# DeepMETv2/DeepMETv2

Measured on AMD Instinct MI355X. Metric: events/sec (4.5k PF cands, k=16), higher is better.
Workload: dtype f32

## Files before the change

deepmetv2_amd/_lib.py:

```python
from __future__ import annotations

import ctypes as C
import os
import threading

_PKG_DIR = os.path.dirname(os.path.abspath(__file__))
LIB_PATH = os.environ.get("DMET_HIP_LIB") or os.path.join(_PKG_DIR, "libdmet_hip.so")

_lock = threading.Lock()
_lib = None

_vp, _i, _i64, _sz, _f, _d = C.c_void_p, C.c_int, C.c_int64, C.c_size_t, C.c_float, C.c_double

SIGNATURES = {
    "dmet_version": (_i, []),
    "dmet_last_error": (C.c_char_p, []),
    "dmet_device_available": (_i, []),
    "dmet_knn_workspace_bytes": (_sz, [_i64, _i, _i, _i]),
    "dmet_knn_f32": (_i, [_vp, _vp, _i, _i64, _i, _i, _vp, _vp, _vp, _sz, _vp]),
    "dmet_knn_local_f32": (_i, [_vp, _vp, _i, _i64, _i, _i, _vp, _vp, _vp, _vp, _sz, _vp]),
    "dmet_knn_periodic_f32": (_i, [_vp, _vp, _i, _i64, _i, _i, _vp, _vp, _vp, _vp, _vp, _sz, _vp]),
    "dmet_knn_xy_workspace_bytes": (_sz, [_i64, _i64, _i, _i, _i]),
    "dmet_knn_xy_f32": (_i, [_vp, _vp, _i64, _vp, _vp, _i64, _i, _i, _i, _vp, _vp, _vp, _vp, _sz, _vp]),
    "dmet_radius_xy_f32": (_i, [_vp, _vp, _i64, _vp, _vp, _i64, _i, _i, _f, _i, _vp, _i, _vp, _vp, _vp]),
    "dmet_edge_features_xy_f32": (_i, [_vp, _vp, _vp, _vp, _i64, _i, _vp, _vp]),
    "dmet_edge_features_xy_bwd_f32": (_i, [_vp, _vp, _vp, _vp, _i64, _i64, _i, _vp, _vp, _vp]),
    "dmet_adamw_f32": (_i, [_vp, _vp, _vp, _vp, _vp, _vp, _i64, _d, _d, _d, _d, _d, _vp]),
    "dmet_adamw_lr_f32": (_i, [_vp, _vp, _vp, _vp, _vp, _vp, _i64, _vp, _d, _d, _d, _d, _vp]),
    "dmet_bn_knn_local_dense_f32": (_i, [_vp, _vp, _vp, _vp, _vp, _vp, _vp, _vp, _i, _i64, _i, _i, _vp, _vp, _vp, _vp, _vp, _i,
                                         _vp, _vp, _vp, _vp, _vp, _sz, _vp]),
    "dmet_knn_local_dense_f32": (_i, [_vp, _vp, _i, _i64, _i, _i, _vp, _vp, _vp, _vp, _vp, _i, _vp, _vp, _vp, _vp, _sz, _vp]),
    "dmet_knn_fallback_stats": (_i, [_vp, _i64, _i, _i, _i, _vp, _vp]),
    "dmet_knn_size_hint": (_i, [_i, _i]),
    "dmet_finalize_defer_begin": (_i, []),
    "dmet_finalize_pending": (_i, []),
    "dmet_finalize_flush": (_i, [_vp]),
    "dmet_radius_f32": (_i, [_vp, _vp, _i, _i64, _i, _f, _i, _i, _vp, _vp, _vp]),
    "dmet_radius_counted_f32": (_i, [_vp, _vp, _i, _i64, _i, _f, _i, _i, _vp, _vp, _vp]),
    "dmet_radius_workspace_bytes": (_sz, [_i64]),
    "dmet_radius_windowed_f32": (_i, [_vp, _vp, _i, _i64, _i, _f, _i, _i, _i, _vp, _vp, _vp, _sz, _vp]),
    "dmet_radius_windowed_local_f32": (_i, [_vp, _vp, _i, _i64, _i, _f, _i, _i, _i, _vp, _vp, _vp, _i, _vp, _sz, _vp]),
    "dmet_radius_periodic_f32": (_i, [_vp, _vp, _i, _i64, _i, _f, _i, _i, _i, _vp, _vp, _vp, _vp]),
    "dmet_radius_windowed_periodic_f32": (_i, [_vp, _vp, _i, _i64, _i, _f, _i, _i, _i, _vp, _vp, _vp, _vp, _i, _vp, _sz,
                                               _vp]),
    "dmet_edgeconv_linear_workspace_bytes": (_sz, [_i64, _i]),
    "dmet_edgeconv_linear_max_fwd_f32": (_i, [_vp, _vp, _vp, _i, _i64, _i, _i, _i, _vp, _vp, _vp, _vp, _vp, _sz, _vp]),
    "dmet_edgeconv_fused_lds_f32": (_i, [_vp, _vp, _vp, _i, _i64, _i, _i, _i, _vp, _vp, _vp, _vp, _vp]),
    "dmet_node_linear_split_f32": (_i, [_vp, _i64, _i, _i, _vp, _vp, _vp, _vp, _vp]),
    "dmet_node_linear_split_sliced_f32": (_i, [_vp, _i64, _i, _i, _vp, _vp, _vp, _vp, _vp]),
    "dmet_bn_node_linear_split_f32": (_i, [_vp, _vp, _vp, _vp, _vp, _vp, _vp, _i64, _i, _vp, _vp, _i, _vp, _vp, _vp]),
    "dmet_gather_max_f32": (_i, [_vp, _vp, _vp, _vp, _i, _i64, _i, _i, _vp, _vp, _vp]),
    "dmet_gather_max_counted_f32": (_i, [_vp, _vp, _vp, _vp, _i64, _i, _i, _vp, _vp, _vp]),
    "dmet_gather_max_lds_f32": (_i, [_vp, _vp, _vp, _vp, _i, _i64, _i, _i, _vp, _vp, _vp]),
    "dmet_gather_max_counted_lds_f32": (_i, [_vp, _vp, _vp, _vp, _vp, _i, _i64, _i, _i, _i, _vp, _vp, _vp]),
    "dmet_gather_max_lds_sliced_f32": (_i, [_vp, _vp, _vp, _vp, _vp, _i, _i64, _i, _i, _vp, _vp, _vp]),
    "dmet_gather_max_lds_sliced_cap_f32": (_i, [_vp, _vp, _vp, _vp, _vp, _i, _i64, _i, _i, _vp, _vp, _i64, _vp]),
    "dmet_gather_max_lds16_f32": (_i, [_vp, _vp, _vp, _vp, _vp, _i, _i64, _i, _i, _vp, _vp, _vp]),
    "dmet_edge_mlp2_supported": (_i, [_i, _i, _i, _i]),
    "dmet_edge_mlp2_bf16": (_i, [_vp, _i64, _i, _vp, _i, _vp, _vp, _i, _vp, _vp, _i, _i, _i, _vp, _vp]),
    "dmet_edge_mlp2_bn_workspace_bytes": (_sz, [_i64, _i]),
    "dmet_edge_mlp2_bn_bf16": (_i, [_vp, _i64, _i, _vp, _i, _vp, _vp, _i, _vp, _vp, _i, _i, _i, _vp, _vp, _f, _f, _vp, _vp, _vp,
                                    _i, _vp, _vp, _sz, _vp]),
    "dmet_edge_mlp_f32_supported": (_i, [_i, _i, _i]),
    "dmet_edge_mlp_f32_workspace_bytes": (_sz, [_i64, _i64, _i, _i, _i]),
    "dmet_edge_mlp_fwd_f32": (_i, [_vp, _i64, _i, _vp, _vp, _vp, _i64, _vp, _vp, _i, _vp, _vp, _i, _i, _i, _i, _vp, _vp, _f, _f,
# ... 121 lines not shown
```

deepmetv2_amd/_native.py:

```python
from __future__ import annotations

import contextlib
import ctypes
import inspect
import os
from typing import Optional, Tuple

import torch

from . import _lib


def _require_device(*tensors: torch.Tensor) -> torch.device:
    dev = None
    for t in tensors:
        if t is None:
            continue
        if t.device.type != "cuda":
            raise RuntimeError(
                "deepmetv2_amd: operator called with a non-GPU tensor. The HIP extension is the only "
                "implementation (no CPU fallback); move inputs to a ROCm device.")
        if dev is None:
            dev = t.device
        elif t.device != dev:
# ... 164 lines not shown
        dense = None

    def call(nbr, dist, loc_p, ws):
        if dense is None:
            _lib.check(L.dmet_knn_local_f32(x.data_ptr(), ptr.data_ptr(), B, N, D, k, nbr.data_ptr(), dist.data_ptr(),
                                            loc_p, ws.data_ptr(), ws.numel(), _stream(dev)), "dmet_knn_local_f32")
            return None
        W, b, sliced = dense
        W = _f32c(W.detach(), "W")
        bp = _f32c(b.detach(), "b").data_ptr() if b is not None else None
        if sliced == "bf16":
            Pt = torch.empty((N, 32), dtype=torch.float32, device=dev)
            Qt = torch.empty((N, 32), dtype=torch.bfloat16, device=dev)
            layout = 2
        else:
            PQ = torch.empty((2, 4, N, 8) if sliced else (2, N, 32), dtype=torch.float32, device=dev)
            Pt, Qt = PQ[0], PQ[1]
            layout, sliced = (1 if sliced else 0), bool(sliced)
        done = ctypes.c_int(0)
        _lib.check(L.dmet_knn_local_dense_f32(x.data_ptr(), ptr.data_ptr(), B, N, D, k, nbr.data_ptr(),
                                              dist.data_ptr(), loc_p, W.data_ptr(), bp, layout, Pt.data_ptr(),
                                              Qt.data_ptr(), ctypes.cast(ctypes.pointer(done), ctypes.c_void_p),
                                              ws.data_ptr(), ws.numel(), _stream(dev)), "dmet_knn_local_dense_f32")
        return (Pt, Qt, sliced) if done.value else None

    nbr, dist, loc, ws, pq = _knn_run(dev, N, k, want_local, L.dmet_knn_workspace_bytes(N, B, D, k), call)
    if stats is not None and N > 0 and B > 0:
        with _on(dev):
            out = (ctypes.c_int64 * 2)()
            _lib.check(L.dmet_knn_fallback_stats(ws.data_ptr(), N, B, D, k, ctypes.cast(out, ctypes.c_void_p),
                                                 _stream(dev)), "dmet_knn_fallback_stats")
            stats["flagged_tiles"], stats["flagged_queries"] = int(out[0]), int(out[1])
            stats["tiles"] = (N + 127) // 128
    if asked:
        return nbr, dist, loc, pq
    return nbr, dist, loc


def knn(x: torch.Tensor, ptr: torch.Tensor, k: int, stats: Optional[dict] = None) -> Tuple[torch.Tensor, torch.Tensor]:
    nbr, dist, _ = _knn(x, ptr, k, stats, False)
    return nbr, dist


def knn_local_dense(x: torch.Tensor, ptr: torch.Tensor, k: int, W: torch.Tensor, b: Optional[torch.Tensor],
                    sliced, stats: Optional[dict] = None):
    out = _knn(x, ptr, k, stats, True, dense=(W, b, sliced))
    return out if len(out) == 4 else (*out, None)


def knn_local(x: torch.Tensor, ptr: torch.Tensor, k: int, stats: Optional[dict] = None
              ) -> Tuple[torch.Tensor, torch.Tensor, torch.Tensor]:
    return _knn(x, ptr, k, stats, True)


def _period_array(period, D: int):
    if period is None:
        return None, None
    if len(period) != D:
        raise ValueError(f"period has {len(period)} entries for {D} coordinates")
    per = (ctypes.c_float * D)(*[float(p) for p in period])
    return per, ctypes.cast(per, ctypes.c_void_p)


def knn_periodic(x: torch.Tensor, ptr: torch.Tensor, k: int, period, want_local: bool):
    dev, x, N, D, B = _knn_operands(x, ptr)
    L = _lib.load()
# ... 1569 lines not shown
```

deepmetv2_amd/csrc/knn.hip:

```cpp
#include <stdlib.h>

#include "common.h"
#include "knn_common.h"
#include "nls_body.h"

namespace dmet {
namespace {

constexpr int kTileC = 32;
constexpr int kQMax = 8;
constexpr int kMaxSplit = 8;
constexpr int kWavesPerGroup = 4;

#define DMET_PKSUB_LO " op_sel:[0,0] op_sel_hi:[0,1] neg_lo:[0,1] neg_hi:[0,1]\n\t"
#define DMET_PKSUB_HI " op_sel:[1,0] op_sel_hi:[1,1] neg_lo:[0,1] neg_hi:[0,1]\n\t"
__device__ __forceinline__ void pk_dist_step4(f2 &accA, f2 &accB, f2 vxy, f2 vzw, f2 wxy, f2 wzw, f2 q0, f2 q1, f2 q2,
                                              f2 q3)
{
    f2 t0, t1, t2, t3;
    asm("v_pk_add_f32 %[t0], %[vxy], %[q0]" DMET_PKSUB_LO
        "v_pk_add_f32 %[t1], %[wxy], %[q0]" DMET_PKSUB_LO
        "v_pk_add_f32 %[t2], %[vxy], %[q1]" DMET_PKSUB_HI
        "v_pk_add_f32 %[t3], %[wxy], %[q1]" DMET_PKSUB_HI
        "v_pk_fma_f32 %[a], %[t0], %[t0], %[a]\n\t"
// ... 824 lines not shown
        w.fplan = reinterpret_cast<KnnPlan *>(take(sizeof(KnnPlan)));
        w.forder = reinterpret_cast<int32_t *>(take(sizeof(int32_t) * ((size_t)B + 1)));
        w.fpos_of = reinterpret_cast<int32_t *>(take(sizeof(int32_t) * ((size_t)B + 1)));
        w.ftile_ptr = reinterpret_cast<int32_t *>(take(sizeof(int32_t) * ((size_t)B + 1)));
        w.nrm = reinterpret_cast<float *>(take(sizeof(float) * (size_t)N));
        w.nrec = (N >> 5) + B + 1;
        w.rec = reinterpret_cast<uint8_t *>(take((size_t)w.nrec * kRecBytesMax));
        w.zero_bytes = sizeof(int32_t) * ((size_t)exact_tiles_max(N, B) + 4) + (size_t)N;
        w.flags = reinterpret_cast<int32_t *>(take(w.zero_bytes));
        w.any = w.flags + exact_tiles_max(N, B);
        w.qflag = reinterpret_cast<uint8_t *>(w.any + 4);
        w.qlist = reinterpret_cast<int32_t *>(take(sizeof(int32_t) * (size_t)N));
    }
    w.bytes = (size_t)(p - reinterpret_cast<uintptr_t>(ws));
    return w;
}

inline int filter_mode()
{
    const char *e = getenv("DMET_KNN_PATH");
    if (e && strcmp(e, "exact") == 0) return 0;
#if defined(DMET_KNN_EXPERIMENT) || defined(DMET_FILTER_ABL) || defined(DMET_F2_ABL) || defined(DMET_F2_SAMEREC)
    if (e && strcmp(e, "filter_only") == 0) return 2;
#endif
    return 1;
}

inline int filter_form2()
{
    const char *e = getenv("DMET_KNN_FILTER");
    return (e && strcmp(e, "1") == 0) ? 0 : 1;
}

template <int KF, int NH = 1>
int launch_filter(const KnnFilterArgs &f, const KnnWorkspace &w, int simds, const KnnPlanOut &px, const KnnPlanOut &pf,
                  hipStream_t st, const KnnRider *rider, const KnnAffine *affine)
{
    const int slots = simds * kF2WavesPerSimd;
    if (affine) {
        if constexpr (NH == 1)
            hipLaunchKernelGGL((knn_prep_kernel<1, true>), dim3((unsigned)((w.nrec * kWave + 255) / 256 + 2)), dim3(256), 0, st, f.x,
                               f.ptr, f.B, f.N, w.nrm, w.rec, w.nrec, reinterpret_cast<uint32_t *>(w.flags), w.zero_bytes, px,
                               pf, f.form2, *affine);
    } else {
        hipLaunchKernelGGL((knn_prep_kernel<NH>), dim3((unsigned)((w.nrec * kWave + 255) / 256 + 2)), dim3(256), 0, st, f.x,
                           f.ptr, f.B, f.N, w.nrm, w.rec, w.nrec, reinterpret_cast<uint32_t *>(w.flags), w.zero_bytes, px, pf,
                           f.form2, KnnAffine{});
    }
    DMET_LAUNCH_CHECK("knn_prep_kernel");
    const int64_t ftiles_max = (f.N + kFQ - 1) / kFQ + f.B;
    const int64_t fblocks = (ftiles_max + slots + kWavesPerGroup - 1) / kWavesPerGroup;
    if (f.form2) {
        KnnFilterArgs fr = f;
        int64_t grid = fblocks;
        if (rider) {
            fr.rW = rider->W; fr.rb = rider->b; fr.rP = rider->P; fr.rQ = rider->Q; fr.r_sliced = rider->sliced;
            fr.first_rider = (int)fblocks;
            grid = fblocks + rider_groups();
        }
        hipLaunchKernelGGL((knn_filter12_kernel<KF, NH>), dim3((unsigned)grid), dim3(kWave * kWavesPerGroup), 0, st, fr);
        DMET_LAUNCH_CHECK("knn_filter12_kernel");
    } else {
        if constexpr (NH == 1) hipLaunchKernelGGL((knn_filter_kernel<KF>), dim3((unsigned)fblocks), dim3(kWave * kWavesPerGroup), 0, st, f);
        DMET_LAUNCH_CHECK("knn_filter_kernel");
    }
    constexpr int kRerankQpb = 4 * (kWave / filter_list_len(KF));
// ... 29 lines not shown

template <int DP, int KP>
KnnOutcome launch_knn(const KnnBuild &r, const KnnWorkspace &w)
{
    KnnOutcome done;
    constexpr int TQ = (DP <= 32) ? 2 : 1;
    constexpr int QT = kWave * TQ;
    const KnnQuerySet *qs = r.qs.qx ? &r.qs : nullptr;
    int simds = num_simds();
    if (simds > kMaxSimds) simds = kMaxSimds;
    bool use_filter = false;
    if constexpr ((DP == 32 || DP == 64) && KP <= 32)
        use_filter = !qs && r.D == DP && r.k <= 20 && aligned16(r.x) && filter_mode() != 0 && (DP == 32 || filter_form2());
    constexpr int NH = DP == 64 ? 2 : 1;
    const int slots = simds * kF2WavesPerSimd;
    const KnnPlanOut px{QT, simds, kMaxSplit, w.order, w.pos_of, w.tile_ptr, w.plan};
    const KnnPlanOut pf{kFQ, slots, kFilterMaxSplit, w.forder, w.fpos_of, w.ftile_ptr, w.fplan};
    if (qs) {
        hipLaunchKernelGGL(knn_plan_xy_kernel, dim3(1), dim3(256), 0, r.st, qs->qptr, r.ptr, r.B, px);
        DMET_LAUNCH_CHECK("knn_plan_xy_kernel");
    } else if (!use_filter) {
        hipLaunchKernelGGL(knn_plan_kernel, dim3(1), dim3(256), 0, r.st, r.ptr, r.B, px, pf);
        DMET_LAUNCH_CHECK("knn_plan_kernel");
    }
    KnnArgs a{r.x, r.ptr, r.B, r.N, r.D, r.k, r.nbr, r.dist, r.nbr16, w.wsd, w.wsj, w.plan, w.order, w.tile_ptr, w.psd, w.psj,
              nullptr, 0, nullptr, nullptr, nullptr, 0, QT};
    if (!qs && !use_filter && hipMemsetAsync(w.flags, 0, w.zero_bytes, r.st) != hipSuccess)
        return hip_fail(hipGetLastError(), "hipMemsetAsync");

    if (use_filter) {
        KnnFilterArgs f{r.x, r.ptr, r.B, r.N, r.k, w.nrm, w.rec, w.fplan, w.forder, w.fpos_of, w.ftile_ptr,
                        w.psd, w.psj, r.nbr, r.dist, r.nbr16, w.flags, w.any, w.qflag, w.qlist, w.tile_ptr, QT, filter_form2(),
                        NH == 1 ? 1.0f : 1.5f, nullptr, nullptr, nullptr, nullptr, 0, 0,
                        (aligned16(r.nbr) && aligned16(r.dist) && aligned16(r.nbr16) && !env_is("DMET_KNN_EMIT", "lanes")) ? 1 : 0, 0};
        f.no_rerank = (f.form2 && r.hint.min_nodes >= kF2MinNodes && r.hint.max_nodes >= r.hint.min_nodes &&
                       r.hint.max_nodes <= kF2MaxNodes) ? 1 : 0;
        const KnnAffine *affine = (NH == 1 && r.affine.raw) ? &r.affine : nullptr;
        const KnnRider *rider = (NH == 1 && f.form2 && r.rider.P) ? &r.rider : nullptr;
        int rc = 0;
        if constexpr (DP == 32 || DP == 64) {
            if constexpr (KP == 8) rc = launch_filter<8, NH>(f, w, simds, px, pf, r.st, rider, affine);
            else if constexpr (KP == 16) rc = launch_filter<16, NH>(f, w, simds, px, pf, r.st, rider, affine);
            else if constexpr (KP == 32) rc = launch_filter<20, NH>(f, w, simds, px, pf, r.st, rider, affine);
        }
        if (rc) return rc;
        done.affine_done = affine != nullptr;
        done.rider_done = rider != nullptr;
        if (filter_mode() == 2) return done;
        a.flags = w.flags;
        a.any = w.any;
        if constexpr (NH == 1) {
            a.qlist = w.qlist;
            a.pos_of = w.pos_of;
            a.requery_groups = kRequeryGroups;
            a.flag_min = kRequeryMax + 1;
        } else {
            a.flag_min = 1;
        }
    }

    const int64_t tiles_max = (r.N + QT - 1) / QT + r.B;
    const int64_t blocks = (tiles_max + simds + kWavesPerGroup - 1) / kWavesPerGroup + a.requery_groups;
    unsigned dyn = 0;
#ifdef DMET_KNN_EXPERIMENT
    if (const char *e = getenv("DMET_KNN_EXTRA_LDS")) dyn = (unsigned)atoi(e);
#endif
    const bool exact_d = r.D == DP && aligned16(r.x) && (!qs || aligned16(qs->qx));
// ... 173 lines not shown
    }
    *fused = (o.rc == 0) ? 1 : 0;
    return o.rc;
}

extern "C" int dmet_knn_fallback_stats(const void *ws, int64_t N, int B, int D, int k, int64_t *out, dmet_stream_t stream)
{
    (void)D;
    DMET_REQUIRE(N > 0 && B > 0 && k >= 1 && k <= DMET_MAX_K && ws && out, "dmet_knn_fallback_stats: bad arguments");
    const KnnWorkspace w = carve_workspace(const_cast<void *>(ws), N, B, padded_k(k));
    const int64_t n = exact_tiles_max(N, B);
    int32_t *host = static_cast<int32_t *>(malloc(sizeof(int32_t) * (size_t)n));
    DMET_REQUIRE(host != nullptr, "dmet_knn_fallback_stats: out of host memory");
    hipStream_t st = as_stream(stream);
    hipError_t e = hipMemcpyAsync(host, w.flags, sizeof(int32_t) * (size_t)n, hipMemcpyDeviceToHost, st);
    if (e == hipSuccess) e = hipStreamSynchronize(st);
    if (e != hipSuccess) { free(host); return hip_fail(e, "dmet_knn_fallback_stats"); }
    out[0] = 0; out[1] = 0;
    for (int64_t i = 0; i < n; ++i) { out[0] += host[i] != 0; out[1] += host[i]; }
    free(host);
    if (getenv("DMET_KNN_LIST_FLAGGED") && out[1] > 0) {
        int32_t ids[16];
        const int64_t m = out[1] < 16 ? out[1] : 16;
        if (hipMemcpy(ids, w.qlist, sizeof(int32_t) * (size_t)m, hipMemcpyDeviceToHost) == hipSuccess)
            for (int64_t i = 0; i < m; ++i) {
                uint8_t why = 0;
                (void)hipMemcpy(&why, w.qflag + ids[i], 1, hipMemcpyDeviceToHost);
                fprintf(stderr, "[dmet] flagged query %d (qflag %d)\n", ids[i], (int)why);
            }
    }
    return 0;
}

extern "C" size_t dmet_knn_xy_workspace_bytes(int64_t Nx, int64_t Ny, int B, int D, int k)
{
    (void)Nx; (void)D;
    if (Ny <= 0 || B < 0 || k <= 0 || k > DMET_MAX_K) return 0;
    return carve_workspace(nullptr, Ny, B, padded_k(k), true).bytes + 512;
}

extern "C" int dmet_knn_xy_f32(const float *x, const int64_t *ptr_x, int64_t Nx, const float *y, const int64_t *ptr_y,
                               int64_t Ny, int B, int D, int k, const float *period, int32_t *nbr, float *dist, void *ws,
                               size_t ws_bytes, dmet_stream_t stream)
{
    const int64_t kMaxRows = (int64_t)2147483647 - 4096;
    DMET_REQUIRE(Nx >= 0 && Nx < kMaxRows && Ny >= 0 && Ny < kMaxRows, "dmet_knn_xy_f32: Nx=%lld / Ny=%lld out of range",
                 (long long)Nx, (long long)Ny);
    DMET_REQUIRE(B >= 0, "dmet_knn_xy_f32: B=%d", B);
    DMET_REQUIRE(k >= 1 && k <= DMET_MAX_K, "dmet_knn_xy_f32: k=%d not in [1,%d]", k, DMET_MAX_K);
    DMET_REQUIRE(D >= 1 && D <= DMET_MAX_KNN_DIM, "dmet_knn_xy_f32: D=%d not in [1,%d]", D, DMET_MAX_KNN_DIM);
    RadPeriod per;
    bool any = false;
    if (period) {
        const int rc = radius_periods("dmet_knn_xy_f32", D, period, &per, &any);
        if (rc) return rc;
    }
    if (Ny == 0) return 0;
    DMET_REQUIRE(B >= 1, "dmet_knn_xy_f32: %lld queries but no event", (long long)Ny);
    DMET_REQUIRE((x || Nx == 0) && ptr_x && y && ptr_y && nbr && dist && ws, "dmet_knn_xy_f32: null pointer");
    DMET_REQUIRE(ws_bytes >= dmet_knn_xy_workspace_bytes(Nx, Ny, B, D, k), "dmet_knn_xy_f32: workspace too small");
    return knn_build(KnnBuild{x, ptr_x, Ny, KnnQuerySet{y, ptr_y}, any ? &per : nullptr, B, D, k, nbr, dist, nullptr, ws,
                              ws_bytes, as_stream(stream), KnnRider{}, KnnAffine{}, KnnSizeHint{}}).rc;
}
```

deepmetv2_amd/csrc/knn_filter.h:

```cpp
constexpr int kFQ = 64;

typedef float f32x16 __attribute__((ext_vector_type(16)));
typedef short bf16x8 __attribute__((ext_vector_type(8)));
typedef _Float16 f16x8 __attribute__((ext_vector_type(8)));

struct KnnFilterArgs {
    const float *x;
    const int64_t *ptr;
    int B;
    int64_t N;
    int k;
    float *nrm;
    uint8_t *rec;
    const KnnPlan *plan;
    const int32_t *order;
    const int32_t *pos_of;
    const int32_t *tile_ptr;
    float *psd;
    int32_t *psj;
    int32_t *nbr;
    float *dist;
    uint16_t *nbr16;
    int32_t *flags;
    int32_t *any;
    uint8_t *qflag;
    int32_t *qlist;
    const int32_t *xtile_ptr;
    int xtile_queries;
    int form2;
    float slack_scale;
    const float *rW, *rb;
    float *rP, *rQ;
    int r_sliced;
    int first_rider;
    int emit_coalesced;
    int no_rerank;
};

struct KnnRider {
    const float *W = nullptr, *b = nullptr;
    float *P = nullptr, *Q = nullptr;
    int sliced = 0;
};

struct KnnAffine {
    const float *raw = nullptr, *res = nullptr, *gamma = nullptr, *beta = nullptr, *mean = nullptr, *invstd = nullptr;
    int kernarg_pad = 0;
};
static_assert(sizeof(KnnAffine) == 56, "KnnAffine is the tail of knn_prep_kernel's argument block: keep its size");

inline int rider_groups()
{
    static int cached = 0;
    if (cached == 0) {
        const char *e = getenv("DMET_KNN_RIDER_GROUPS");
        const int v = e ? atoi(e) : 0;
        cached = (v >= 1 && v <= 4096) ? v : 512;
    }
    return cached;
}

__device__ __forceinline__ void flag_query(const KnnFilterArgs &a, int q, int xtile)
{
    a.qflag[q] = 1;
    atomicAdd(a.flags + xtile, 1);
    const int slot = atomicAdd(a.any, 1);
    if (slot < a.N) a.qlist[slot] = q;
}

// ... 682 lines not shown

__device__ __forceinline__ unsigned f2_tau16(float tau, float &rep)
{
    const float x = __builtin_amdgcn_fmed3f(-tau * (1.0f / kF2TauC[0]), -65504.0f, 65504.0f);
    float v = __builtin_amdgcn_fmed3f(__builtin_fmaf(__builtin_fabsf(x), -0x1p-9f, x), -65504.0f, 65504.0f);
    const float y0 = (float)__builtin_amdgcn_cvt_pkrtz(v, v)[0];
    const float w = __builtin_fmaf(-y0, kF2TauC[0] / kF2TauC[1], x * (kF2TauC[0] / kF2TauC[1]));
    v = fminf(__builtin_fmaf(__builtin_fabsf(w), -0x1p-9f, w - 0x1p-24f), 65504.0f);
    const auto y = __builtin_amdgcn_cvt_pkrtz(y0, v);
    rep = -__builtin_fmaf(y0, kF2TauC[0], (float)y[1] * kF2TauC[1]);
    return __builtin_bit_cast(unsigned, y);
}

__device__ __forceinline__ float f2_key_lower(float cmin, float rep)
{
    const float s = cmin + rep;
    return __builtin_fmaf(__builtin_fabsf(s), -0x1p-22f, __builtin_fmaf(__builtin_fabsf(rep), -0x1p-17f, s));
}

template <int NH = 1>
__device__ __forceinline__ float f2_cert_T(float tau)
{
    if constexpr (NH != 1) return tau;
    const float T = fminf(tau, kF2TauRepMax);
    return __builtin_fmaf(__builtin_fabsf(T), -0x1p-16f, T) - 1e-16f;
}
template <int NH = 1>
__device__ __forceinline__ bool f2_full(float tau) { return NH == 1 || tau < kKnnSentinel; }

__device__ __forceinline__ float f2_slack(float an, float rn, float scale)
{
    return 2.0f * scale * (4e-5f * an * rn + 1e-5f * rn * rn + 4e-6f * an * an) + 1.96e-3f * an * rn + 6e-7f * (an + rn) +
           6e-14f * rn * rn + 1e-12f;
}

constexpr int f2_list_len(int KP) { return KP <= 16 ? KP + 6 : KP + 4; }

__device__ __forceinline__ int f2_mask_row(int p) { return (p & 3) + 8 * ((p & 15) >> 2) + 4 * (p >> 4); }

template <int M, bool UPD, bool REC, bool INS, int NH = 1, bool CONV = true, int LEAD = 2>
__device__ __forceinline__ void f2_tile(F2Lane<M> &L, F2Wave &S, const uint8_t *__restrict__ rec, int64_t rbase, int t,
                                        int t_hi, f32x16 &c0, f32x16 &c1, f32x16 &n0, f32x16 &n1, float &rc, float &rn,
                                        const F2Ops<NH> &use, F2Ops<NH> &ld, const f16x8 (&bq)[2][2 * NH], int lane,
                                        int hh, bool alive, float &carry)
{
#if defined(DMET_F2_ABL) && DMET_F2_ABL >= 2
    constexpr bool kRec = false;
#else
    constexpr bool kRec = REC;
#endif
#if defined(DMET_F2_ABL) && DMET_F2_ABL >= 3
    constexpr bool kUpd = false;
#else
    constexpr bool kUpd = UPD;
#endif
    if (kRec) {
        if (__any(L.cnt >= kF2Slots - 1)) f2_compact<M>(L, S, lane, kF2Slots - 3);
    }
#if defined(DMET_F2_SAMEREC)
    f2_load<NH>(ld, rec, rbase + (t & 1), lane, hh);
#else
    f2_load<NH>(ld, rec, rbase + min(t + LEAD, t_hi - 1), lane, hh);
#endif
    {
        unsigned q0 = 0u, q1 = 0u;
        if (NH == 1 && kRec) {
// ... 128 lines not shown
__device__ __forceinline__ void filter2_wave(const KnnFilterArgs &a, F2Wave &S, int *tickets, int group, int wv, int lane)
{
    constexpr int M = f2_list_len(KP);
    constexpr int D = 32 * NH;
    constexpr int MS = (M + 1 + 3) & ~3;
    const int col = lane & 31, hh = lane >> 5;
    const uint8_t *__restrict__ rec = a.rec;
    const int64_t *__restrict__ ptr = a.ptr;

    const int n_full = a.plan->n_full, split = a.plan->split, total = a.plan->total_tiles;
    const int item = group * kWavesPerGroup + wv;
    int tile = item, sub = 0, nsub = 1;
    if (item >= n_full) {
        const int r = item - n_full;
        tile = n_full + r / split;
        sub = r % split;
        nsub = split;
    }
    if (tile >= total) return;
    const int pos = find_tile_event(a.tile_ptr, a.B, tile);
    const int ev = a.order[pos];
    const int ev_lo = (int)ptr[ev], ev_hi = (int)ptr[ev + 1];
    const int q_first = ev_lo + (tile - a.tile_ptr[pos]) * kFQ;
    if (!f2_in_domain(ev_hi - ev_lo)) {
        if (NH != 1 && sub == 0) {
            const int q = q_first + lane;
            if (q < ev_hi) {
                flag_query(a, q, a.xtile_ptr[pos] + (q - ev_lo) / a.xtile_queries);
            }
        }
        return;
    }
    int clo = ev_lo, chi = ev_hi;
    bool idle_piece = false;
    if (nsub > 1) {
        if (ev_hi - ev_lo < kF2SplitMinNodes) {
            idle_piece = sub != 0;
        } else {
            const int chunk = (((chi - clo) + nsub - 1) / nsub + 31) & ~31;
            clo = min(chi, clo + sub * chunk);
            chi = min(chi, clo + chunk);
        }
    }
    const int64_t rbase = (ptr[ev] >> 5) + ev;
    const int64_t rlast = rbase + (ev_hi - ev_lo - 1) / 32;
    const int t_lo = (clo - ev_lo) / 32, t_hi = idle_piece ? t_lo : (chi - ev_lo + 31) / 32;

    const int myq = q_first + hh * 32 + col;
    const bool valid = myq < ev_hi;
    float t_fix = -__builtin_inff();
    bool act = valid;
    for (int attempt = 0;; ++attempt) {
    F2Lane<M> L;
#pragma unroll
    for (int p = 0; p < M; ++p) L.tk[p] = kKnnSentinel;
    L.tau = attempt == 0 ? -__builtin_inff() : t_fix;
    L.tq = 0u;
    L.rep = 0.0f;
    L.cnt = 0;
    L.overflow = false;
    {
        f16x8 bq[2][2 * NH];
#pragma unroll
        for (int b = 0; b < 2; ++b) {
            const int64_t qrec = min(rbase + (q_first - ev_lo) / 32 + b, rlast);
            const f16x8 *g = reinterpret_cast<const f16x8 *>(rec + qrec * rec_bytes(NH));
#pragma unroll
            for (int m = 0; m < 2 * NH; ++m) bq[b][m] = g[m * 64 + lane] * (_Float16)-2.0f;
        }
        if (attempt == 0) {
            const int t_def = min(t_hi, t_lo + kF2Defer);
            f2_sweep<M, true, false, NH>(L, S, rec, rbase, t_lo, t_def, bq, lane, hh, valid);
            f2_sweep<M, true, true, NH>(L, S, rec, rbase, t_def, t_hi, bq, lane, hh, valid);
            f2_sweep<M, false, true, NH>(L, S, rec, rbase, t_lo, t_def, bq, lane, hh, valid);
        } else {
            f2_sweep<M, false, true, NH>(L, S, rec, rbase, t_lo, t_hi, bq, lane, hh, valid);
        }
    }
    f2_compact<M>(L, S, lane, kF2Slots);
#if defined(DMET_F2_ABL) && DMET_F2_ABL >= 1
    return;
#endif

    const int64_t qrow_id = valid ? myq : ev_lo;
    float qrow[D];
    {
        const float4 *g = reinterpret_cast<const float4 *>(a.x + qrow_id * D);
#pragma unroll
        for (int c = 0; c < D / 4; ++c) {
            const float4 v = g[c];
            qrow[4 * c] = v.x; qrow[4 * c + 1] = v.y; qrow[4 * c + 2] = v.z; qrow[4 * c + 3] = v.w;
        }
    }
    unsigned long long kk[KP];
#pragma unroll
    for (int p = 0; p < KP; ++p) kk[p] = (unsigned long long)__float_as_uint(kKnnSentinel) << 32;
    const int nent = (act && !L.overflow) ? L.cnt : 0;
    int slot = 0;
    unsigned cmask = 0u;
    int ctile = 0;
    auto pop = [&]() __attribute__((always_inline)) -> int32_t {
        if (cmask == 0u && slot < nent) {
            const uint2 e = S.ent[slot][lane];
            cmask = e.x;
            ctile = (int)(e.y & kF2TileMask);
            ++slot;
// ... 135 lines not shown
            if (!__any(ja >= 0)) break;
            jc = pop(); pc = fetch(jc);
            round(pa, ja);
            if (!__any(jb >= 0)) break;
            ja = pop(); pa = fetch(ja);
            round(pb, jb);
            if (!__any(jc >= 0)) break;
            jb = pop(); pb = fetch(jb);
            round(pc, jc);
        }
    } else {
        int32_t ja = pop(), jb;
        HalfRows pa = fetch(ja), pb;
        for (;;) {
            if (!__any(ja >= 0)) break;
            jb = pop(); pb = fetch(jb);
            round(pa, ja);
            if (!__any(jb >= 0)) break;
            ja = pop(); pa = fetch(ja);
            round(pb, jb);
        }
    }
    }
#ifdef DMET_RR_PRIO
    __builtin_amdgcn_s_setprio(0);
#endif
    float kd[KP];
    int32_t kj[KP];
#pragma unroll
    for (int p = 0; p < KP; ++p) {
        kd[p] = __uint_as_float((unsigned)(kk[p] >> 32));
        kj[p] = kd[p] == kKnnSentinel ? -1 : (int32_t)(unsigned)kk[p];
    }
    const int k = a.k;
    const float tau = attempt == 0 ? L.tk[M - 1] : t_fix;
    auto emit = [&](const bool rows_on, const bool coop) __attribute__((always_inline)) -> float {
        float kth = -1.0f;
#pragma unroll
        for (int p = 0; p < KP; ++p)
            if (p == k - 1 && kj[p] >= 0) kth = kd[p];
        if constexpr (KP % 4 == 0 && KP <= 20) {
            if (coop && a.emit_coalesced && k == KP) {
                constexpr int RP = KP / 4;
                const unsigned long long on = __ballot(rows_on);
                unsigned *stg = reinterpret_cast<unsigned *>(&S);
                const int64_t blk = (int64_t)q_first * KP;
                wave_sync();
#pragma unroll
                for (int q = 0; q < RP; ++q)
                    *reinterpret_cast<uint4 *>(stg + lane * KP + 4 * q) =
                        make_uint4((unsigned)kj[4 * q], (unsigned)kj[4 * q + 1], (unsigned)kj[4 * q + 2], (unsigned)kj[4 * q + 3]);
                wave_sync();
#pragma unroll
                for (int t = 0; t < RP; ++t) {
                    const int pi = t * 64 + lane;
                    const uint4 v = *reinterpret_cast<const uint4 *>(stg + 4 * pi);
                    if ((on >> (pi / RP)) & 1ull) *reinterpret_cast<uint4 *>(a.nbr + blk + 4 * pi) = v;
                }
                wave_sync();
#pragma unroll
                for (int q = 0; q < RP; ++q)
                    *reinterpret_cast<uint4 *>(stg + lane * KP + 4 * q) =
                        make_uint4(__float_as_uint(kd[4 * q]), __float_as_uint(kd[4 * q + 1]), __float_as_uint(kd[4 * q + 2]),
                                   __float_as_uint(kd[4 * q + 3]));
                wave_sync();
#pragma unroll
                for (int t = 0; t < RP; ++t) {
                    const int pi = t * 64 + lane;
                    const uint4 v = *reinterpret_cast<const uint4 *>(stg + 4 * pi);
                    if ((on >> (pi / RP)) & 1ull) *reinterpret_cast<uint4 *>(a.dist + blk + 4 * pi) = v;
                }
                if (a.nbr16) {
                    if constexpr (KP % 8 == 0) {
                        constexpr int RH = KP / 8;
                        wave_sync();
#pragma unroll
                        for (int q = 0; q < RH; ++q) {
                            uint4 w;
                            w.x = (unsigned)local_id16(kj[8 * q], ev_lo) | ((unsigned)local_id16(kj[8 * q + 1], ev_lo) << 16);
                            w.y = (unsigned)local_id16(kj[8 * q + 2], ev_lo) | ((unsigned)local_id16(kj[8 * q + 3], ev_lo) << 16);
                            w.z = (unsigned)local_id16(kj[8 * q + 4], ev_lo) | ((unsigned)local_id16(kj[8 * q + 5], ev_lo) << 16);
                            w.w = (unsigned)local_id16(kj[8 * q + 6], ev_lo) | ((unsigned)local_id16(kj[8 * q + 7], ev_lo) << 16);
                            *reinterpret_cast<uint4 *>(stg + lane * (KP / 2) + 4 * q) = w;
                        }
                        wave_sync();
#pragma unroll
                        for (int t = 0; t < RH; ++t) {
                            const int pi = t * 64 + lane;
                            const uint4 v = *reinterpret_cast<const uint4 *>(stg + 4 * pi);
                            if ((on >> (pi / RH)) & 1ull)
                                *reinterpret_cast<uint4 *>(reinterpret_cast<unsigned *>(a.nbr16 + blk) + 4 * pi) = v;
                        }
                    } else if (rows_on) {
                        uint16_t *r16 = a.nbr16 + (int64_t)myq * k;
#pragma unroll
                        for (int p = 0; p + 1 < KP; p += 2)
                            reinterpret_cast<unsigned *>(r16)[p >> 1] =
                                (unsigned)local_id16(kj[p], ev_lo) | ((unsigned)local_id16(kj[p + 1], ev_lo) << 16);
                    }
                }
                wave_sync();
                return kth;
            }
        }
        if (!rows_on) return kth;
#pragma unroll
        for (int p = 0; p < KP; ++p) {
            if (p < k) {
                a.nbr[(int64_t)myq * k + p] = kj[p];
                a.dist[(int64_t)myq * k + p] = kd[p];
            }
        }
        if (a.nbr16) {
            uint16_t *r16 = a.nbr16 + (int64_t)myq * k;
            if ((k & 1) == 0) {
#pragma unroll
                for (int p = 0; p + 1 < KP; p += 2)
                    if (p < k)
                        reinterpret_cast<unsigned *>(r16)[p >> 1] =
                            (unsigned)local_id16(kj[p], ev_lo) | ((unsigned)local_id16(kj[p + 1], ev_lo) << 16);
            } else {
#pragma unroll
                for (int p = 0; p < KP; ++p)
                    if (p < k) r16[p] = local_id16(kj[p], ev_lo);
            }
        }
        return kth;
    };
    if (nsub == 1) {
        bool retry = false;
        const float kth = emit(act, true);
        if (act) {
            const float nx = a.nrm[myq];
            const float an = __builtin_sqrtf(nx) * 1.000001f;
            const float rn = an + __builtin_sqrtf(fmaxf(kth, 0.0f)) * 1.00002f;
            const float slack = f2_slack(an, rn, NH == 1 ? 1.0f : 1.5f);
            const bool wideq = !(nx < kF16WideLimit * kF16WideLimit);
            const bool fail = L.overflow || wideq || (f2_full<NH>(tau) && !(kth >= 0.0f && f2_cert_T<NH>(tau) + nx - slack > kth));
            float ts = kth - nx + slack;
            ts += __builtin_fabsf(ts) * ((NH == 1 ? 0x1p-15f : 0.0f) + 4.8e-7f) + (nx + slack) * 4.8e-7f + (NH == 1 ? 2e-16f : 1e-30f);
            retry = fail && attempt == 0 && !L.overflow && !wideq && kth >= 0.0f && f2_cert_T<NH>(ts) + nx - slack > kth &&
                    ts < kKnnSentinel;
            if (fail && !retry) {
                flag_query(a, myq, a.xtile_ptr[pos] + (myq - ev_lo) / a.xtile_queries);
#ifdef DMET_KNN_WHY
                a.qflag[myq] = (uint8_t)(1 | (L.overflow ? 2 : 0) | (wideq ? 4 : 0) | (kth < 0.0f ? 8 : 0) | (attempt ? 16 : 0) |
                                         (!(ts < kKnnSentinel) ? 32 : 0) | (!(f2_cert_T<NH>(ts) + nx - slack > kth) ? 64 : 0));
                a.dist[(int64_t)myq * k + 0] = tau; a.dist[(int64_t)myq * k + 1] = kth; a.dist[(int64_t)myq * k + 2] = slack; a.dist[(int64_t)myq * k + 3] = (float)L.cnt;
#endif
            }
            t_fix = retry ? ts : -__builtin_inff();
        }
        if (!__any(retry)) return;
        act = retry;
        continue;
    }
    static_assert(kFilterMaxSplit == 2 && kWavesPerGroup % 2 == 0, "pairs of sub-sweeps share a workgroup");
    const int64_t fslot = (int64_t)(tile - n_full) * kFQ + hh * 32 + col;
    if (valid) {
        float *ld = a.psd + (fslot * nsub + sub) * MS;
        int32_t *lj = a.psj + (fslot * nsub + sub) * MS;
#pragma unroll
        for (int p = 0; p < KP; ++p) { ld[p] = kd[p]; lj[p] = kj[p]; }
        ld[M] = tau;
        lj[M] = L.overflow ? 1 : 0;
    }
    __builtin_amdgcn_fence(__ATOMIC_RELEASE, "workgroup");
    int arrived = 0;
    if (lane == 0) arrived = atomicAdd(&tickets[wv >> 1], 1);
    arrived = __builtin_amdgcn_readfirstlane(arrived);
    if (arrived == 0) return;
    __builtin_amdgcn_fence(__ATOMIC_ACQUIRE, "workgroup");
    float tau_o = kKnnSentinel;
    int of_o = 0;
    if (valid) {
        const float *ld = a.psd + (fslot * nsub + (sub ^ 1)) * MS;
        const int32_t *lj = a.psj + (fslot * nsub + (sub ^ 1)) * MS;
        tau_o = ld[M];
        of_o = lj[M];
#pragma unroll
        for (int p = 0; p < KP; ++p) {
            const float od = ld[p];
            const int32_t oj = lj[p];
            const unsigned long long nk = oj >= 0 ? (((unsigned long long)__float_as_uint(od) << 32) | (unsigned)oj) : ~0ull;
            bool g[KP];
#pragma unroll
            for (int q = 0; q < KP; ++q) g[q] = kk[q] > nk;
#pragma unroll
            for (int q = KP - 1; q >= 1; --q) kk[q] = g[q - 1] ? kk[q - 1] : (g[q] ? nk : kk[q]);
            kk[0] = g[0] ? nk : kk[0];
        }
#pragma unroll
        for (int p = 0; p < KP; ++p) {
            kd[p] = __uint_as_float((unsigned)(kk[p] >> 32));
            kj[p] = kd[p] == kKnnSentinel ? -1 : (int32_t)(unsigned)kk[p];
        }
        const float kth = emit(true, false);
        const float nx = a.nrm[myq];
        const float an = __builtin_sqrtf(nx) * 1.000001f;
        const float rn = an + __builtin_sqrtf(fmaxf(kth, 0.0f)) * 1.00002f;
        const float slack = f2_slack(an, rn, NH == 1 ? 1.0f : 1.5f);
        const bool wideq = !(nx < kF16WideLimit * kF16WideLimit);
        const bool fail_a = f2_full<NH>(tau) && !(kth >= 0.0f && f2_cert_T<NH>(tau) + nx - slack > kth);
        const bool fail_b = f2_full<NH>(tau_o) && !(kth >= 0.0f && f2_cert_T<NH>(tau_o) + nx - slack > kth);
        if (L.overflow || of_o != 0 || wideq || fail_a || fail_b)
            flag_query(a, myq, a.xtile_ptr[pos] + (myq - ev_lo) / a.xtile_queries);
    }
    return;
    }
}

template <int KP, int NH = 1>
__global__ __launch_bounds__(kWave * kWavesPerGroup, kF2WavesPerSimd) void knn_filter12_kernel(const KnnFilterArgs a)
{
    union WaveLds {
        F2Wave f2;
#ifndef DMET_F2_LEAN
        FilterQueue<filter_queue_len(filter_list_len(KP))> f1;
#endif
    };
    __shared__ WaveLds sh_all[kWavesPerGroup];
    if constexpr (NH == 1) {
        if (a.rP != nullptr && (int)blockIdx.x >= a.first_rider) {
            static_assert(sizeof(WaveLds) >= sizeof(float) * kNlsLdsFloats, "a wavefront's LDS holds the transposition tiles");
            const int rwv = __builtin_amdgcn_readfirstlane(threadIdx.x >> 6);
            const int64_t wave = (int64_t)((int)blockIdx.x - a.first_rider) * kWavesPerGroup + rwv;
            const int64_t nwaves = (int64_t)((int)gridDim.x - a.first_rider) * kWavesPerGroup;
            float *tp = reinterpret_cast<float *>(&sh_all[rwv]);
            if (a.r_sliced == 2)
                node_linear_split_bf16_wave<32, 32>(a.x, a.N, a.rW, a.rb, a.rP, reinterpret_cast<unsigned short *>(a.rQ), wave,
                                                    nwaves, threadIdx.x & 63);
            else if (a.r_sliced == 1) node_linear_split_wave<32, 32, true>(a.x, a.N, a.rW, a.rb, a.rP, a.rQ, tp, wave, nwaves, threadIdx.x & 63);
            else node_linear_split_wave<32, 32, false>(a.x, a.N, a.rW, a.rb, a.rP, a.rQ, tp, wave, nwaves, threadIdx.x & 63);
            return;
        }
    }
    static_assert(sizeof(WaveLds) == sizeof(F2Wave), "the union is sized by the second form");
#ifndef DMET_F2_LEAN
    static_assert(sizeof(FilterQueue<filter_queue_len(filter_list_len(KP))>) <= sizeof(F2Wave) - 8, "ticket bytes are free");
// ... 135 lines not shown
```

include/dmet.h:

```cpp
#ifndef DMET_H_
#define DMET_H_

#include <stddef.h>
#include <stdint.h>

#ifdef __cplusplus
extern "C" {
#endif

typedef void *dmet_stream_t;

#define DMET_VERSION 1
#define DMET_MAX_K 64
#define DMET_MAX_KNN_DIM 64
#define DMET_MAX_H 128

int dmet_version(void);
const char *dmet_last_error(void);
int dmet_device_available(void);

size_t dmet_knn_workspace_bytes(int64_t N, int B, int D, int k);
int dmet_knn_f32(const float *x, const int64_t *ptr, int B, int64_t N, int D, int k, int32_t *nbr,
                 float *dist, void *ws, size_t ws_bytes, dmet_stream_t stream);
int dmet_knn_local_f32(const float *x, const int64_t *ptr, int B, int64_t N, int D, int k, int32_t *nbr,
                       float *dist, uint16_t *nbr_local, void *ws, size_t ws_bytes, dmet_stream_t stream);
int dmet_knn_periodic_f32(const float *x, const int64_t *ptr, int B, int64_t N, int D, int k, const float *period,
                          int32_t *nbr, float *dist, uint16_t *nbr_local, void *ws, size_t ws_bytes,
                          dmet_stream_t stream);
size_t dmet_knn_xy_workspace_bytes(int64_t Nx, int64_t Ny, int B, int D, int k);
int dmet_knn_xy_f32(const float *x, const int64_t *ptr_x, int64_t Nx, const float *y, const int64_t *ptr_y, int64_t Ny,
                    int B, int D, int k, const float *period, int32_t *nbr, float *dist, void *ws, size_t ws_bytes,
                    dmet_stream_t stream);
int dmet_knn_local_dense_f32(const float *x, const int64_t *ptr, int B, int64_t N, int D, int k, int32_t *nbr,
                             float *dist, uint16_t *nbr_local, const float *W, const float *bias, int layout,
                             float *P, void *Q, int *dense_done, void *ws, size_t ws_bytes, dmet_stream_t stream);
int dmet_bn_knn_local_dense_f32(const float *raw, const float *residual, const float *gamma, const float *beta,
                                const float *mean, const float *invstd, float *y, const int64_t *ptr, int B, int64_t N,
                                int D, int k, int32_t *nbr, float *dist, uint16_t *nbr_local, const float *W,
                                const float *bias, int layout, float *P, void *Q, int *dense_done, int *fused, void *ws,
                                size_t ws_bytes, dmet_stream_t stream);

int dmet_knn_size_hint(int min_nodes, int max_nodes);

int dmet_knn_fallback_stats(const void *ws, int64_t N, int B, int D, int k, int64_t *out, dmet_stream_t stream);

int dmet_radius_f32(const float *x, const int64_t *ptr, int B, int64_t N, int D, float r, int max_nbr, int skip_self,
                    int32_t *nbr, int32_t *cnt, dmet_stream_t stream);
int dmet_radius_counted_f32(const float *x, const int64_t *ptr, int B, int64_t N, int D, float r, int max_nbr,
                            int skip_self, int32_t *nbr, int32_t *cnt, dmet_stream_t stream);
size_t dmet_radius_workspace_bytes(int64_t N);
int dmet_radius_windowed_f32(const float *x, const int64_t *ptr, int B, int64_t N, int D, float r, int max_nbr,
                             int skip_self, int fill, int32_t *nbr, int32_t *cnt, void *ws, size_t ws_bytes,
                             dmet_stream_t stream);
int dmet_radius_windowed_local_f32(const float *x, const int64_t *ptr, int B, int64_t N, int D, float r, int max_nbr,
                                   int skip_self, int fill, int32_t *nbr, int32_t *cnt, uint16_t *nbr16, int stride16,
                                   void *ws, size_t ws_bytes, dmet_stream_t stream);
int dmet_radius_periodic_f32(const float *x, const int64_t *ptr, int B, int64_t N, int D, float r, int max_nbr,
                             int skip_self, int fill, const float *period, int32_t *nbr, int32_t *cnt,
                             dmet_stream_t stream);
int dmet_radius_windowed_periodic_f32(const float *x, const int64_t *ptr, int B, int64_t N, int D, float r, int max_nbr,
                                      int skip_self, int fill, const float *period, int32_t *nbr, int32_t *cnt,
                                      uint16_t *nbr16, int stride16, void *ws, size_t ws_bytes, dmet_stream_t stream);
int dmet_radius_xy_f32(const float *x, const int64_t *ptr_x, int64_t Nx, const float *y, const int64_t *ptr_y, int64_t Ny,
                       int B, int D, float r, int max_nbr, const float *period, int fill, int32_t *nbr, int32_t *cnt,
                       dmet_stream_t stream);

size_t dmet_edgeconv_linear_workspace_bytes(int64_t N, int Hout);
int dmet_edgeconv_linear_max_fwd_f32(const float *x, const int32_t *nbr, const int64_t *ptr, int B,
                                     int64_t N, int k, int Hin, int Hout, const float *W,
                                     const float *b, float *out, uint8_t *arg, void *ws,
                                     size_t ws_bytes, dmet_stream_t stream);
int dmet_edgeconv_fused_lds_f32(const float *x, const int32_t *nbr, const int64_t *ptr, int B, int64_t N, int k,
                                int Hin, int Hout, const float *W, const float *b, float *out, uint8_t *arg,
                                dmet_stream_t stream);
int dmet_node_linear_split_f32(const float *x, int64_t N, int Hin, int Hout, const float *W,
                               const float *b, float *P, float *Q, dmet_stream_t stream);
int dmet_gather_max_f32(const float *P, const float *Q, const int32_t *nbr, const int64_t *ptr, int B,
// ... 270 lines not shown
```

Before: 47930.

## Tighten f2 filter threshold after deferred sweep using a scaled certificate cut

After the deferred first sweep in the form-2 kNN filter, each query computes a cut threshold from its current k-th distance and norm, scaled by a configurable factor (default 1.25), and lowers tau to it. This prunes candidates in the second sweep so less distance work and list insertion is done, with the risk of more certification failures and retries. Small split pieces now exit early instead of running idle, emission uses pinned lane/query registers, and retry counters are added via atomics with a new stats entry point.

Result: faster. 48500 (median of 6 runs) (+1.2%).

```diff
diff --git a/deepmetv2_amd/_lib.py b/deepmetv2_amd/_lib.py
--- a/deepmetv2_amd/_lib.py
+++ b/deepmetv2_amd/_lib.py
@@ -31,6 +31,7 @@
                                          _vp, _vp, _vp, _vp, _vp, _sz, _vp]),
     "dmet_knn_local_dense_f32": (_i, [_vp, _vp, _i, _i64, _i, _i, _vp, _vp, _vp, _vp, _vp, _i, _vp, _vp, _vp, _vp, _sz, _vp]),
     "dmet_knn_fallback_stats": (_i, [_vp, _i64, _i, _i, _i, _vp, _vp]),
+    "dmet_knn_retry_stats": (_i, [_vp, _i64, _i, _i, _i, _vp, _vp]),
     "dmet_knn_size_hint": (_i, [_i, _i]),
     "dmet_finalize_defer_begin": (_i, []),
     "dmet_finalize_pending": (_i, []),
diff --git a/deepmetv2_amd/_native.py b/deepmetv2_amd/_native.py
--- a/deepmetv2_amd/_native.py
+++ b/deepmetv2_amd/_native.py
@@ -220,6 +220,9 @@
                                                  _stream(dev)), "dmet_knn_fallback_stats")
             stats["flagged_tiles"], stats["flagged_queries"] = int(out[0]), int(out[1])
             stats["tiles"] = (N + 127) // 128
+            _lib.check(L.dmet_knn_retry_stats(ws.data_ptr(), N, B, D, k, ctypes.cast(out, ctypes.c_void_p),
+                                              _stream(dev)), "dmet_knn_retry_stats")
+            stats["second_attempts"], stats["second_attempt_queries"] = int(out[0]), int(out[1])
     if asked:
         return nbr, dist, loc, pq
     return nbr, dist, loc
diff --git a/deepmetv2_amd/csrc/knn.hip b/deepmetv2_amd/csrc/knn.hip
--- a/deepmetv2_amd/csrc/knn.hip
+++ b/deepmetv2_amd/csrc/knn.hip
@@ -880,6 +880,17 @@
     return (e && strcmp(e, "1") == 0) ? 0 : 1;
 }
 
+constexpr float kF2CutScale = 1.25f;
+inline float knn_cut_scale()
+{
+    const char *e = getenv("DMET_KNN_CUT");
+    if (!e || !*e) return kF2CutScale;
+    if (strcmp(e, "0") == 0 || strcmp(e, "off") == 0) return -1.0f;
+    char *end = nullptr;
+    const float v = strtof(e, &end);
+    return (end != e && *end == '\0' && v >= 0.0f && v <= 1e6f) ? v : kF2CutScale;
+}
+
 template <int KF, int NH = 1>
 int launch_filter(const KnnFilterArgs &f, const KnnWorkspace &w, int simds, const KnnPlanOut &px, const KnnPlanOut &pf,
                   hipStream_t st, const KnnRider *rider, const KnnAffine *affine)
@@ -975,7 +986,8 @@
         KnnFilterArgs f{r.x, r.ptr, r.B, r.N, r.k, w.nrm, w.rec, w.fplan, w.forder, w.fpos_of, w.ftile_ptr,
                         w.psd, w.psj, r.nbr, r.dist, r.nbr16, w.flags, w.any, w.qflag, w.qlist, w.tile_ptr, QT, filter_form2(),
                         NH == 1 ? 1.0f : 1.5f, nullptr, nullptr, nullptr, nullptr, 0, 0,
-                        (aligned16(r.nbr) && aligned16(r.dist) && aligned16(r.nbr16) && !env_is("DMET_KNN_EMIT", "lanes")) ? 1 : 0, 0};
+                        (aligned16(r.nbr) && aligned16(r.dist) && aligned16(r.nbr16) && !env_is("DMET_KNN_EMIT", "lanes")) ? 1 : 0, 0,
+                        knn_cut_scale(), w.any + 1};
         f.no_rerank = (f.form2 && r.hint.min_nodes >= kF2MinNodes && r.hint.max_nodes >= r.hint.min_nodes &&
                        r.hint.max_nodes <= kF2MaxNodes) ? 1 : 0;
         const KnnAffine *affine = (NH == 1 && r.affine.raw) ? &r.affine : nullptr;
@@ -1215,6 +1227,21 @@
     return 0;
 }
 
+extern "C" int dmet_knn_retry_stats(const void *ws, int64_t N, int B, int D, int k, int64_t *out, dmet_stream_t stream)
+{
+    (void)D;
+    DMET_REQUIRE(N > 0 && B > 0 && k >= 1 && k <= DMET_MAX_K && ws && out, "dmet_knn_retry_stats: bad arguments");
+    const KnnWorkspace w = carve_workspace(const_cast<void *>(ws), N, B, padded_k(k));
+    int32_t host[2] = {0, 0};
+    hipStream_t st = as_stream(stream);
+    hipError_t e = hipMemcpyAsync(host, w.any + 1, sizeof(host), hipMemcpyDeviceToHost, st);
+    if (e == hipSuccess) e = hipStreamSynchronize(st);
+    if (e != hipSuccess) return hip_fail(e, "dmet_knn_retry_stats");
+    out[0] = host[0];
+    out[1] = host[1];
+    return 0;
+}
+
 extern "C" size_t dmet_knn_xy_workspace_bytes(int64_t Nx, int64_t Ny, int B, int D, int k)
 {
     (void)Nx; (void)D;
diff --git a/deepmetv2_amd/csrc/knn_filter.h b/deepmetv2_amd/csrc/knn_filter.h
--- a/deepmetv2_amd/csrc/knn_filter.h
+++ b/deepmetv2_amd/csrc/knn_filter.h
@@ -35,6 +35,8 @@
     int first_rider;
     int emit_coalesced;
     int no_rerank;
+    float cut_scale;
+    int32_t *retries;
 };
 
 struct KnnRider {
@@ -783,6 +785,27 @@
 {
     return 2.0f * scale * (4e-5f * an * rn + 1e-5f * rn * rn + 4e-6f * an * an) + 1.96e-3f * an * rn + 6e-7f * (an + rn) +
            6e-14f * rn * rn + 1e-12f;
+}
+
+template <int NH = 1>
+__device__ __forceinline__ float f2_cert_threshold(float kth, float nx, float slack)
+{
+    float ts = kth - nx + slack;
+    ts += __builtin_fabsf(ts) * ((NH == 1 ? 0x1p-15f : 0.0f) + 4.8e-7f) + (nx + slack) * 4.8e-7f + (NH == 1 ? 2e-16f : 1e-30f);
+    return ts;
+}
+
+template <int NH = 1>
+__device__ __forceinline__ float f2_cut(float tkk, float nx, float scale)
+{
+    const float sc = NH == 1 ? 1.0f : 1.5f;
+    const float an = __builtin_sqrtf(nx) * 1.000001f;
+    const float u0 = fmaxf(tkk + nx, 0.0f);
+    float s = f2_slack(an, an + __builtin_sqrtf(u0) * 1.00002f, sc);
+    s = f2_slack(an, an + __builtin_sqrtf(u0 + s) * 1.00002f, sc);
+    const float U = u0 + s;
+    const float ts = f2_cert_threshold<NH>(U, nx, f2_slack(an, an + __builtin_sqrtf(U) * 1.00002f, sc));
+    return __builtin_fmaf(scale, ts - tkk, tkk);
 }
 
 constexpr int f2_list_len(int KP) { return KP <= 16 ? KP + 6 : KP + 4; }
@@ -977,10 +1000,10 @@
         return;
     }
     int clo = ev_lo, chi = ev_hi;
-    bool idle_piece = false;
     if (nsub > 1) {
         if (ev_hi - ev_lo < kF2SplitMinNodes) {
-            idle_piece = sub != 0;
+            if (sub != 0) return;
+            nsub = 1;
         } else {
             const int chunk = (((chi - clo) + nsub - 1) / nsub + 31) & ~31;
             clo = min(chi, clo + sub * chunk);
@@ -989,7 +1012,7 @@
     }
     const int64_t rbase = (ptr[ev] >> 5) + ev;
     const int64_t rlast = rbase + (ev_hi - ev_lo - 1) / 32;
-    const int t_lo = (clo - ev_lo) / 32, t_hi = idle_piece ? t_lo : (chi - ev_lo + 31) / 32;
+    const int t_lo = (clo - ev_lo) / 32, t_hi = (chi - ev_lo + 31) / 32;
 
     const int myq = q_first + hh * 32 + col;
     const bool valid = myq < ev_hi;
@@ -1017,6 +1040,18 @@
             const int t_def = min(t_hi, t_lo + kF2Defer);
             f2_sweep<M, true, false, NH>(L, S, rec, rbase, t_lo, t_def, bq, lane, hh, valid);
             f2_sweep<M, true, true, NH>(L, S, rec, rbase, t_def, t_hi, bq, lane, hh, valid);
+            if (a.cut_scale >= 0.0f) {
+                float tkk = kKnnSentinel;
+#pragma unroll
+                for (int p = 0; p < KP; ++p)
+                    if (p == a.k - 1) tkk = L.tk[p];
+                if (tkk < kKnnSentinel) {
+                    int qi = valid ? myq : ev_lo;
+                    asm volatile("" : "+v"(qi));
+                    const float cut = f2_cut<NH>(tkk, a.nrm[qi], a.cut_scale);
+                    L.tau = fminf(L.tau, cut);
+                }
+            }
             f2_sweep<M, false, true, NH>(L, S, rec, rbase, t_lo, t_def, bq, lane, hh, valid);
         } else {
             f2_sweep<M, false, true, NH>(L, S, rec, rbase, t_lo, t_hi, bq, lane, hh, valid);
@@ -1218,8 +1253,14 @@
         kd[p] = __uint_as_float((unsigned)(kk[p] >> 32));
         kj[p] = kd[p] == kKnnSentinel ? -1 : (int32_t)(unsigned)kk[p];
     }
+    int elane = lane, eq = myq;
+#ifdef DMET_F2_PIN32
+    asm volatile("" : "+v"(elane), "+v"(eq));
+#else
+    if constexpr (NH != 1) asm volatile("" : "+v"(elane), "+v"(eq));
+#endif
     const int k = a.k;
-    const float tau = attempt == 0 ? L.tk[M - 1] : t_fix;
+    const float tau = L.tau;
     auto emit = [&](const bool rows_on, const bool coop) __attribute__((always_inline)) -> float {
         float kth = -1.0f;
 #pragma unroll
@@ -1234,25 +1275,25 @@
                 wave_sync();
 #pragma unroll
                 for (int q = 0; q < RP; ++q)
-                    *reinterpret_cast<uint4 *>(stg + lane * KP + 4 * q) =
+                    *reinterpret_cast<uint4 *>(stg + elane * KP + 4 * q) =
                         make_uint4((unsigned)kj[4 * q], (unsigned)kj[4 * q + 1], (unsigned)kj[4 * q + 2], (unsigned)kj[4 * q + 3]);
                 wave_sync();
 #pragma unroll
                 for (int t = 0; t < RP; ++t) {
-                    const int pi = t * 64 + lane;
+                    const int pi = t * 64 + elane;
                     const uint4 v = *reinterpret_cast<const uint4 *>(stg + 4 * pi);
                     if ((on >> (pi / RP)) & 1ull) *reinterpret_cast<uint4 *>(a.nbr + blk + 4 * pi) = v;
                 }
                 wave_sync();
 #pragma unroll
                 for (int q = 0; q < RP; ++q)
-                    *reinterpret_cast<uint4 *>(stg + lane * KP + 4 * q) =
+                    *reinterpret_cast<uint4 *>(stg + elane * KP + 4 * q) =
                         make_uint4(__float_as_uint(kd[4 * q]), __float_as_uint(kd[4 * q + 1]), __float_as_uint(kd[4 * q + 2]),
                                    __float_as_uint(kd[4 * q + 3]));
                 wave_sync();
 #pragma unroll
                 for (int t = 0; t < RP; ++t) {
-                    const int pi = t * 64 + lane;
+                    const int pi = t * 64 + elane;
                     const uint4 v = *reinterpret_cast<const uint4 *>(stg + 4 * pi);
                     if ((on >> (pi / RP)) & 1ull) *reinterpret_cast<uint4 *>(a.dist + blk + 4 * pi) = v;
                 }
@@ -1267,18 +1308,18 @@
                             w.y = (unsigned)local_id16(kj[8 * q + 2], ev_lo) | ((unsigned)local_id16(kj[8 * q + 3], ev_lo) << 16);
                             w.z = (unsigned)local_id16(kj[8 * q + 4], ev_lo) | ((unsigned)local_id16(kj[8 * q + 5], ev_lo) << 16);
                             w.w = (unsigned)local_id16(kj[8 * q + 6], ev_lo) | ((unsigned)local_id16(kj[8 * q + 7], ev_lo) << 16);
-                            *reinterpret_cast<uint4 *>(stg + lane * (KP / 2) + 4 * q) = w;
+                            *reinterpret_cast<uint4 *>(stg + elane * (KP / 2) + 4 * q) = w;
                         }
                         wave_sync();
 #pragma unroll
                         for (int t = 0; t < RH; ++t) {
-                            const int pi = t * 64 + lane;
+                            const int pi = t * 64 + elane;
                             const uint4 v = *reinterpret_cast<const uint4 *>(stg + 4 * pi);
                             if ((on >> (pi / RH)) & 1ull)
                                 *reinterpret_cast<uint4 *>(reinterpret_cast<unsigned *>(a.nbr16 + blk) + 4 * pi) = v;
                         }
                     } else if (rows_on) {
-                        uint16_t *r16 = a.nbr16 + (int64_t)myq * k;
+                        uint16_t *r16 = a.nbr16 + (int64_t)eq * k;
 #pragma unroll
                         for (int p = 0; p + 1 < KP; p += 2)
                             reinterpret_cast<unsigned *>(r16)[p >> 1] =
@@ -1293,12 +1334,12 @@
 #pragma unroll
         for (int p = 0; p < KP; ++p) {
             if (p < k) {
-                a.nbr[(int64_t)myq * k + p] = kj[p];
-                a.dist[(int64_t)myq * k + p] = kd[p];
+                a.nbr[(int64_t)eq * k + p] = kj[p];
+                a.dist[(int64_t)eq * k + p] = kd[p];
             }
         }
         if (a.nbr16) {
-            uint16_t *r16 = a.nbr16 + (int64_t)myq * k;
+            uint16_t *r16 = a.nbr16 + (int64_t)eq * k;
             if ((k & 1) == 0) {
 #pragma unroll
                 for (int p = 0; p + 1 < KP; p += 2)
@@ -1317,27 +1358,31 @@
         bool retry = false;
         const float kth = emit(act, true);
         if (act) {
-            const float nx = a.nrm[myq];
+            const float nx = a.nrm[eq];
             const float an = __builtin_sqrtf(nx) * 1.000001f;
             const float rn = an + __builtin_sqrtf(fmaxf(kth, 0.0f)) * 1.00002f;
             const float slack = f2_slack(an, rn, NH == 1 ? 1.0f : 1.5f);
             const bool wideq = !(nx < kF16WideLimit * kF16WideLimit);
             const bool fail = L.overflow || wideq || (f2_full<NH>(tau) && !(kth >= 0.0f && f2_cert_T<NH>(tau) + nx - slack > kth));
-            float ts = kth - nx + slack;
-            ts += __builtin_fabsf(ts) * ((NH == 1 ? 0x1p-15f : 0.0f) + 4.8e-7f) + (nx + slack) * 4.8e-7f + (NH == 1 ? 2e-16f : 1e-30f);
+            const float ts = f2_cert_threshold<NH>(kth, nx, slack);
             retry = fail && attempt == 0 && !L.overflow && !wideq && kth >= 0.0f && f2_cert_T<NH>(ts) + nx - slack > kth &&
                     ts < kKnnSentinel;
             if (fail && !retry) {
-                flag_query(a, myq, a.xtile_ptr[pos] + (myq - ev_lo) / a.xtile_queries);
+                flag_query(a, eq, a.xtile_ptr[pos] + (eq - ev_lo) / a.xtile_queries);
 #ifdef DMET_KNN_WHY
-                a.qflag[myq] = (uint8_t)(1 | (L.overflow ? 2 : 0) | (wideq ? 4 : 0) | (kth < 0.0f ? 8 : 0) | (attempt ? 16 : 0) |
+                a.qflag[eq] = (uint8_t)(1 | (L.overflow ? 2 : 0) | (wideq ? 4 : 0) | (kth < 0.0f ? 8 : 0) | (attempt ? 16 : 0) |
                                          (!(ts < kKnnSentinel) ? 32 : 0) | (!(f2_cert_T<NH>(ts) + nx - slack > kth) ? 64 : 0));
-                a.dist[(int64_t)myq * k + 0] = tau; a.dist[(int64_t)myq * k + 1] = kth; a.dist[(int64_t)myq * k + 2] = slack; a.dist[(int64_t)myq * k + 3] = (float)L.cnt;
+                a.dist[(int64_t)eq * k + 0] = tau; a.dist[(int64_t)eq * k + 1] = kth; a.dist[(int64_t)eq * k + 2] = slack; a.dist[(int64_t)eq * k + 3] = (float)L.cnt;
 #endif
             }
             t_fix = retry ? ts : -__builtin_inff();
         }
         if (!__any(retry)) return;
+        const int nretry = __popcll(__ballot(retry));
+        if (elane == 0) {
+            atomicAdd(a.retries, 1);
+            atomicAdd(a.retries + 1, nretry);
+        }
         act = retry;
         continue;
     }
@@ -1353,7 +1398,7 @@
     }
     __builtin_amdgcn_fence(__ATOMIC_RELEASE, "workgroup");
     int arrived = 0;
-    if (lane == 0) arrived = atomicAdd(&tickets[wv >> 1], 1);
+    if (elane == 0) arrived = atomicAdd(&tickets[wv >> 1], 1);
     arrived = __builtin_amdgcn_readfirstlane(arrived);
     if (arrived == 0) return;
     __builtin_amdgcn_fence(__ATOMIC_ACQUIRE, "workgroup");
@@ -1382,7 +1427,7 @@
             kj[p] = kd[p] == kKnnSentinel ? -1 : (int32_t)(unsigned)kk[p];
         }
         const float kth = emit(true, false);
-        const float nx = a.nrm[myq];
+        const float nx = a.nrm[eq];
         const float an = __builtin_sqrtf(nx) * 1.000001f;
         const float rn = an + __builtin_sqrtf(fmaxf(kth, 0.0f)) * 1.00002f;
         const float slack = f2_slack(an, rn, NH == 1 ? 1.0f : 1.5f);
@@ -1390,7 +1435,7 @@
         const bool fail_a = f2_full<NH>(tau) && !(kth >= 0.0f && f2_cert_T<NH>(tau) + nx - slack > kth);
         const bool fail_b = f2_full<NH>(tau_o) && !(kth >= 0.0f && f2_cert_T<NH>(tau_o) + nx - slack > kth);
         if (L.overflow || of_o != 0 || wideq || fail_a || fail_b)
-            flag_query(a, myq, a.xtile_ptr[pos] + (myq - ev_lo) / a.xtile_queries);
+            flag_query(a, eq, a.xtile_ptr[pos] + (eq - ev_lo) / a.xtile_queries);
     }
     return;
     }
diff --git a/include/dmet.h b/include/dmet.h
--- a/include/dmet.h
+++ b/include/dmet.h
@@ -43,6 +43,7 @@
 int dmet_knn_size_hint(int min_nodes, int max_nodes);
 
 int dmet_knn_fallback_stats(const void *ws, int64_t N, int B, int D, int k, int64_t *out, dmet_stream_t stream);
+int dmet_knn_retry_stats(const void *ws, int64_t N, int B, int D, int k, int64_t *out, dmet_stream_t stream);
 
 int dmet_radius_f32(const float *x, const int64_t *ptr, int B, int64_t N, int D, float r, int max_nbr, int skip_self,
                     int32_t *nbr, int32_t *cnt, dmet_stream_t stream);
```
